# autonomousvision/sdfstudio

Hardware: NVIDIA H100
Metric: rays/sec at 4096 rays x 128 samples (higher is better)
Workload: dtype bf16x3 (fp32 accumulate)

## Files before the change

sdfstudio_b200/csrc/field_tc.h:

```cpp
#pragma once
#include "field_plan.h"

namespace sdfb200 {


constexpr int kEpiWarps = 8;
constexpr int kEpiThreads = kEpiWarps * 32;
constexpr int kTcThreads = kEpiThreads + 128;
constexpr int kEncThreads = 96;
constexpr int kEncItems0 = 288, kEncItems1 = 256, kEncItems2 = 224;
static_assert(kEncItems0 + kEncItems1 + kEncItems2 == 768, "the encoder warps' items cover the tile");
static_assert(kEncItems0 % 32 == 0 && kEncItems1 % 32 == 0, "a warp stages whole 32-row batches (colour_static_tile shuffles across them)");
__host__ __device__ constexpr int enc_item_begin(int w) { return w == 0 ? 0 : w == 1 ? kEncItems0 : w == 2 ? kEncItems0 + kEncItems1 : 768; }
constexpr int kConsumerRegs = 216;
constexpr int kProducerRegs = 72;
static_assert(2 * (kConsumerRegs - 168) <= 168 - kProducerRegs, "setmaxnreg.inc would wait for registers nobody frees");
constexpr int kStages = 5;
constexpr int kKB = 16;
constexpr int kMaxGridDim = 32;
constexpr int kMaxPe = 60;
constexpr int kPeRows = 64;
constexpr int kInK = 96;
constexpr float kHalfPiF = 1.5707963267948966f;
constexpr uint32_t kAPlane = 32 * 2048;
constexpr uint32_t kImgPlane = (kInK / 8) * 128 * 16;
__host__ __device__ constexpr uint32_t tc_stage_bytes(int planes) { return (uint32_t)planes * 256 * kKB * 2; }

enum { PRM_B_G0 = 0, PRM_B_G1, PRM_W_G2 , PRM_B_C0, PRM_B_C1, PRM_W_C2 , kPrmRows = PRM_W_C2 + 3 };
enum { HS_SDF = 0, HS_GRAD , HS_RGB = HS_GRAD + 3 , kHsRows = HS_RGB + 3 };

struct TcSmem { size_t a, ring, prm, hs, coldesc, hx, bytes; };
__host__ __device__ constexpr TcSmem tc_smem(int planes) {
  TcSmem s{};
  s.ring = s.a + (size_t)planes * kAPlane;
  s.prm = s.ring + (size_t)kStages * tc_stage_bytes(planes);
  s.hs = s.prm + kPrmRows * 256 * 4;
  s.coldesc = s.hs + 2 * kHsRows * 128 * 4;
  s.hx = s.coldesc + 96 * 16;
  s.bytes = s.hx + 128 * 8;
  return s;
}
constexpr size_t kSmemPerBlock = 232448;
constexpr size_t kStaticSmem = 1024;
static_assert(tc_smem(2).bytes + kStaticSmem <= kSmemPerBlock, "shared memory of k_field_tc at two planes");

constexpr size_t kFragWords = 64 * 256;
struct TcScratch { size_t sig, h2, slots, slot_bytes, geo, cs, jpe, jg, bytes; };
__host__ __device__ constexpr TcScratch tc_scratch(int planes) {
  TcScratch s{};
  s.h2 = s.sig + kFragWords * 4;
  s.slots = s.h2 + (size_t)planes * kAPlane;
  s.cs = s.geo + (size_t)planes * kImgPlane;
  s.jpe = s.cs + (size_t)planes * kImgPlane;
  s.jg = s.jpe + (size_t)kPeRows * 128 * 4;
  s.slot_bytes = s.jg + (size_t)kMaxGridDim * 3 * 128 * 4;
  s.bytes = s.slots + 2 * s.slot_bytes;
  return s;
}
__host__ __device__ constexpr size_t kScratchPerCta(int planes) { return tc_scratch(planes).bytes; }

__host__ __device__ constexpr int tc_layer_np(int L) { return L == L_B0 ? 128 : 256; }
__host__ __device__ constexpr int tc_layer_k(int L) { return L == L_G0 || L == L_C0MISC ? kInK : 256; }
__host__ __device__ constexpr int tc_layer_kblk(int L) { return kKB * 256 / tc_layer_np(L); }
__host__ __device__ constexpr int tc_layer_nkb(int L) { return tc_layer_k(L) / tc_layer_kblk(L); }
constexpr bool tc_blocks_fill_stages() {
  for (int L = 0; L < L_COUNT; ++L)
    if (tc_layer_np(L) * tc_layer_kblk(L) != 256 * kKB || tc_layer_kblk(L) % 16 != 0 || tc_layer_k(L) % tc_layer_kblk(L) != 0) return false;
  return true;
}
static_assert(tc_blocks_fill_stages(), "every streamed weight block must be one full ring stage of whole K steps");

struct TcLayer {
  unsigned long long w_off;
};

struct TcArgs {
  sdfb200_grid_t grid;
  TcLayer layer[L_COUNT];
// ... 22 lines not shown
```

sdfstudio_b200/csrc/field_tc_kernel.cuh:

```cuda
#pragma once
#include "field_tc.h"
#include "grid.cuh"
#include "tc_common.cuh"

namespace sdfb200 {
using namespace tc;

__device__ __forceinline__ void named_sync(int id, int n) { asm volatile("bar.sync %0, %1;" ::"r"(id), "r"(n) : "memory"); }
constexpr int kEncBar = 3;

struct PointGeom { float px, py, pz, dx, dy, dz, delta, t0, t1; long long ray; };
__device__ __forceinline__ PointGeom point_geom(const TcArgs& a, long long p) {
  PointGeom g;
  g.dx = g.dy = g.dz = 0.f; g.delta = 0.f; g.t0 = g.t1 = 0.f;
  g.ray = a.has_bins ? p / a.n_samples : p;
  if (a.has_bins) {
    const int smp = (int)(p - g.ray * a.n_samples);
    const float t0 = __ldg(a.bins + g.ray * (a.n_samples + 1) + smp);
    g.t0 = t0;
    g.t1 = __ldg(a.bins + g.ray * (a.n_samples + 1) + smp + 1);
    g.delta = __fsub_rn(g.t1, t0);
    g.dx = __ldg(a.directions + g.ray * 3); g.dy = __ldg(a.directions + g.ray * 3 + 1); g.dz = __ldg(a.directions + g.ray * 3 + 2);
    g.px = __fadd_rn(__ldg(a.origins + g.ray * 3 + 0), __fmul_rn(g.dx, t0));
    g.py = __fadd_rn(__ldg(a.origins + g.ray * 3 + 1), __fmul_rn(g.dy, t0));
    g.pz = __fadd_rn(__ldg(a.origins + g.ray * 3 + 2), __fmul_rn(g.dz, t0));
  } else {
    g.px = __ldg(a.origins + p * 3); g.py = __ldg(a.origins + p * 3 + 1); g.pz = __ldg(a.origins + p * 3 + 2);
    if (a.directions) { g.dx = __ldg(a.directions + p * 3); g.dy = __ldg(a.directions + p * 3 + 1); g.dz = __ldg(a.directions + p * 3 + 2); }
  }
  if (a.contraction != SDFB200_CONTRACT_NONE) {
    const float mag = a.contraction == SDFB200_CONTRACT_LINF
                          ? fmaxf(fabsf(g.px), fmaxf(fabsf(g.py), fabsf(g.pz)))
                          : sqrtf(__fadd_rn(__fadd_rn(__fmul_rn(g.px, g.px), __fmul_rn(g.py, g.py)), __fmul_rn(g.pz, g.pz)));
    if (mag >= 1.f) {
      const float k = __fsub_rn(2.f, __fdiv_rn(1.f, mag));
      g.px = __fmul_rn(k, __fdiv_rn(g.px, mag)); g.py = __fmul_rn(k, __fdiv_rn(g.py, mag)); g.pz = __fmul_rn(k, __fdiv_rn(g.pz, mag));
    }
  }
  return g;
}

static __device__ __forceinline__ void sincos_call(float x, float* s, float* c) { sincosf(x, s, c); }
static __device__ __forceinline__ float sin_call(float x) { return sinf(x); }

template <int P, int LAYOUT>
__device__ __forceinline__ void encode_tile_grid(const TcArgs& a, int tile, int row, int grp, uint8_t* img, uint32_t plane, float* Jg,
                                                 uint64_t pol_table) {
  const long long p_raw = (long long)tile * 128 + row;
  const long long p = p_raw < a.n_points ? p_raw : a.n_points - 1;
  const PointGeom g = point_geom(a, p);
  const float x01 = (g.px + 2.0f) * 0.25f, y01 = (g.py + 2.0f) * 0.25f, z01 = (g.pz + 2.0f) * 0.25f;
  const int l_end = min(4 * grp + 4, min(a.grid.n_levels, a.grid.active_levels));
  if (a.use_grid && a.mode != 0) {
#pragma unroll 1
    for (int l = 4 * grp; l < l_end; ++l) {
      LevelCtx c;
      level_prepare<LAYOUT>(a.grid, l, x01, y01, z01, c);
      if (a.grid.table_dtype == SDFB200_DT_F16) level_prefetch_l2<__half, 2>(a.table, c);
      else level_prefetch_l2<float, 2>(a.table, c);
    }
  }
#pragma unroll 1
  for (int l = 4 * grp; l < 4 * grp + 4; ++l) {
    float o[2] = {0.f, 0.f};
    float dj[2][3] = {{0.f, 0.f, 0.f}, {0.f, 0.f, 0.f}};
    if (a.use_grid && l < l_end) {
      LevelCtx c;
      float tv[8][2];
      level_prepare<LAYOUT>(a.grid, l, x01, y01, z01, c);
      if (a.grid.table_dtype == SDFB200_DT_F16) level_fetch<__half, 2, true>(a.table, c, tv, pol_table);
      else level_fetch<float, 2, true>(a.table, c, tv, pol_table);
      level_finish<2, LAYOUT>(a.grid, c, tv, o, dj);
    }
    store_a<P>(img, plane, row, 2 * l, o[0]);
    store_a<P>(img, plane, row, 2 * l + 1, o[1]);
    if (a.mode != 0 && l < a.grid.n_levels) {
#pragma unroll
      for (int f = 0; f < 2; ++f) {
        const int cg = l * 2 + f;
        Jg[(cg * 3 + 0) * 128 + row] = 0.25f * dj[f][0];
        Jg[(cg * 3 + 1) * 128 + row] = 0.25f * dj[f][1];
        Jg[(cg * 3 + 2) * 128 + row] = 0.25f * dj[f][2];
      }
    }
  }
}

template <int P>
__device__ __forceinline__ void encode_tile_pe(const TcArgs& a, int tile, int row, uint8_t* img, uint32_t plane, float* Jpe) {
  const long long p_raw = (long long)tile * 128 + row;
  const long long p = p_raw < a.n_points ? p_raw : a.n_points - 1;
  const PointGeom g = point_geom(a, p);
  if (p_raw < a.n_points) {
    if (a.out.points_norm) a.out.points_norm[p] = sqrtf(__fadd_rn(__fadd_rn(__fmul_rn(g.px, g.px), __fmul_rn(g.py, g.py)), __fmul_rn(g.pz, g.pz)));
    if (a.out.points) { a.out.points[p * 3] = g.px; a.out.points[p * 3 + 1] = g.py; a.out.points[p * 3 + 2] = g.pz; }
  }
  const int deg = a.pe_degree, half = 3 * deg;
  const float pc[3] = {g.px, g.py, g.pz};
  const uint4 z4 = make_uint4(0u, 0u, 0u, 0u);
#pragma unroll 1
  for (int ch = 4; ch < kInK / 8; ++ch) store_a_chunk<P>(img, plane, row, ch, z4, z4);
#pragma unroll 1
  for (int i = 0; i < a.pe_dim; ++i) {
    const int ia = i >= half ? i - half : i;
    const int b = ia / deg, k = ia - b * deg;
    const float fr = (float)(1 << k);
    const float xb = b == 0 ? pc[0] : (b == 1 ? pc[1] : pc[2]);
    const float arg = i >= half ? xb * fr + kHalfPiF : xb * fr;
    float sv, cv;
    sincos_call(arg, &sv, &cv);
    store_a<P>(img, plane, row, 32 + i, a.use_pe ? sv : 0.f);
    if (a.mode != 0) Jpe[i * 128 + row] = a.use_pe ? fr * cv : 0.f;
  }
  store_a<P>(img, plane, row, 32 + a.pe_dim + 0, pc[0]);
  store_a<P>(img, plane, row, 32 + a.pe_dim + 1, pc[1]);
  store_a<P>(img, plane, row, 32 + a.pe_dim + 2, pc[2]);
}

__device__ __forceinline__ float dir_enc(const PointGeom& g, int k) {
  const int i = k < 12 ? k : k - 12, b = i >> 2;
  const float db = b == 0 ? g.dx : (b == 1 ? g.dy : g.dz);
  const float arg = db * (float)(1 << (i & 3));
  return sin_call(k < 12 ? arg : arg + kHalfPiF);
}

template <int P>
__device__ __forceinline__ void colour_static_tile(const TcArgs& a, int tile, int row, uint8_t* img, uint32_t plane) {
  const long long p_raw = (long long)tile * 128 + row;
  const long long p = p_raw < a.n_points ? p_raw : a.n_points - 1;
  const PointGeom g = point_geom(a, p);
  const bool one_ray = __match_any_sync(0xffffffffu, g.ray) == 0xffffffffu;
  const int lane = row & 31;
  const float own = one_ray && lane < 24 ? dir_enc(g, lane) : 0.f;
  const uint4 z4 = make_uint4(0u, 0u, 0u, 0u);
#pragma unroll 1
  for (int ch = 1; ch < kInK / 8; ++ch) store_a_chunk<P>(img, plane, row, ch, z4, z4);
  store_a<P>(img, plane, row, 8 + 0, g.px); store_a<P>(img, plane, row, 8 + 1, g.py); store_a<P>(img, plane, row, 8 + 2, g.pz);
#pragma unroll 1
  for (int k = 0; k < 24; ++k) store_a<P>(img, plane, row, 8 + 3 + k, one_ray ? __shfl_sync(0xffffffffu, own, k) : dir_enc(g, k));
  store_a<P>(img, plane, row, 8 + 27, g.dx); store_a<P>(img, plane, row, 8 + 28, g.dy); store_a<P>(img, plane, row, 8 + 29, g.dz);
  if (a.appearance != nullptr) {
#pragma unroll 1
    for (int j = 0; j < a.app_dim; ++j) store_a<P>(img, plane, row, 8 + 30 + j, __ldg(a.appearance + g.ray * a.app_dim + j));
  }
}

template <int P>
struct Slot {
  uint8_t* base;
  __device__ __forceinline__ Slot(char* slots, uint32_t s) : base(reinterpret_cast<uint8_t*>(slots) + s * tc_scratch(P).slot_bytes) {}
  __device__ __forceinline__ uint8_t* geo() const { return base + tc_scratch(P).geo; }
  __device__ __forceinline__ uint8_t* cs() const { return base + tc_scratch(P).cs; }
  __device__ __forceinline__ float* jpe() const { return reinterpret_cast<float*>(base + tc_scratch(P).jpe); }
  __device__ __forceinline__ float* jg() const { return reinterpret_cast<float*>(base + tc_scratch(P).jg); }
};

#ifdef SDFB200_TC_TIMING
__device__ long long g_tc_timing[16 * 48];
#define TC_PUT(tno, k, v)                                                                                            \
  do {                                                                                                               \
    if (blockIdx.x == 0 && (tno) >= 0 && (tno) < 16) g_tc_timing[(tno) * 48 + (k)] = (v);                            \
  } while (0)
#else
#define TC_PUT(tno, k, v) do { (void)(v); } while (0)
#endif
#define TC_STAMP(k) do { if (tid == 0) TC_PUT(tile_no, k, TC_CLOCK()); } while (0)

struct TcBars {
  Handoff<kStages> ring;
  Handoff<2> enc;
  Handoff<1> a;
  Handoff<2> hs;
  uint64_t cop[2][2];
};

template <int P>
__device__ __forceinline__ void produce_all(const TcArgs& a, int nlayers, uint8_t* abuf, uint8_t* ring, char* slots, TcBars& b) {
  uint32_t j = 0;
// ... 162 lines not shown
    if (c < 3) {
#pragma unroll
      for (int k = 0; k < 16; ++k) sw[k] = sw_next[k];
    }
  }
}

__device__ __forceinline__ float4 col_desc(const TcArgs& a, int ip) {
  const int deg = a.pe_degree, half = 3 * deg;
  int jrow = -1, ax = -1;
  if (ip < a.pe_dim) {
    const int ia = ip >= half ? ip - half : ip;
    ax = ia < deg ? 0 : (ia < 2 * deg ? 1 : 2);
    jrow = ip * 128;
  } else if (ip - a.pe_dim < 3) {
    ax = ip - a.pe_dim;
  }
  return make_float4(__int_as_float(jrow), ax == 0 ? 1.f : 0.f, ax == 1 ? 1.f : 0.f, ax == 2 ? 1.f : 0.f);
}

template <int P>
__device__ __forceinline__ void copy_chunks(uint8_t* abuf, int a_chunk, const uint8_t* src, uint32_t src_plane, int src_chunk, int n, int wrow0,
                                            uint64_t* bar, int lane) {
  for (int k = lane; k < P * n; k += 32) {
    const int pl = k / n, c = k - pl * n;
    bulk_g2s(abuf + pl * kAPlane + (a_chunk + c) * kAChunk + wrow0 * 16, src + pl * src_plane + (src_chunk + c) * kAChunk + wrow0 * 16, 64 * 16, bar);
  }
}
template <int P>
__device__ __forceinline__ void colour_copy(const TileCtx& x, bool early, const uint8_t* cs, uint64_t* bar) {
  constexpr int kMisc = kInK / 8;
  const int lane = x.t & 31;
  if (lane == 0) mbar_arrive_expect_tx(bar, (uint32_t)P * (early ? (kMisc - 1) + kH2Early : 32 - kH2Early) * 64 * 16);
  __syncwarp();
  if (early) {
    copy_chunks<P>(x.abuf, 1, cs, kImgPlane, 1, kMisc - 1, x.wrow0, bar, lane);
    copy_chunks<P>(x.abuf, kMisc, x.h2img, kAPlane, 0, kH2Early, x.wrow0, bar, lane);
  } else {
    copy_chunks<P>(x.abuf, 0, x.h2img, kAPlane, kH2Early, 32 - kH2Early, x.wrow0, bar, lane);
  }
}

template <int P>
__device__ __forceinline__ void epi_eb0(const TileCtx& x, int tile, const Slot<P>& s, const float (&acc)[4][32]) {
  const TcArgs& a = x.a;
  const float* Jpe = s.jpe();
  const float* Jg = s.jg();
  float g0x = 0.f, g0y = 0.f, g0z = 0.f, g1x = 0.f, g1y = 0.f, g1z = 0.f;
#pragma unroll
  for (int c = 0; c < 2; ++c) {
#pragma unroll
    for (int i = 0; i < 32; ++i) {
      const int col = frag_col(x.cq, c, i), row = frag_row(x.r0, i);
      const bool h = frag_half(i);
      float& gx = h ? g1x : g0x;
      float& gy = h ? g1y : g0y;
      float& gz = h ? g1z : g0z;
      const float g = acc[c][i];
      if (c == 0 && i < 16) {
        const bool live = col < a.grid_dim;
        const float* j = Jg + col * 3 * 128 + row;
        const float jx = live ? j[0] : 0.f, jy = live ? j[128] : 0.f, jz = live ? j[256] : 0.f;
        gx = fmaf(g, jx, gx); gy = fmaf(g, jy, gy); gz = fmaf(g, jz, gz);
      } else {
        const float4 d = x.coldesc[col - 32];
        const int jrow = __float_as_int(d.x);
        const float tv = __fmul_rn(g, jrow >= 0 ? Jpe[jrow + row] : 1.f);
        gx = fmaf(tv, d.y, gx); gy = fmaf(tv, d.z, gy); gz = fmaf(tv, d.w, gz);
      }
    }
  }
  g0x = quad_sum(g0x); g0y = quad_sum(g0y); g0z = quad_sum(g0z);
  g1x = quad_sum(g1x); g1y = quad_sum(g1y); g1z = quad_sum(g1z);
  if ((x.t & 3) < 2) {
    const int h = x.t & 1, row = x.r0 + 8 * h;
    const long long p_raw = (long long)tile * 128 + row;
    const PointGeom pg = point_geom(a, p_raw < a.n_points ? p_raw : a.n_points - 1);
    const float grx = h ? g1x : g0x, gry = h ? g1y : g0y, grz = h ? g1z : g0z;
    const float3 n = normalize_eps(grx, gry, grz);
    const float c0v[8] = {grx, gry, grz, a.use_n_dot_v ? n.x * pg.dx + n.y * pg.dy + n.z * pg.dz : 0.f, 0.f, 0.f, 0.f, 0.f};
    store_a_chunk<P>(x.abuf, kAPlane, row, 0, c0v);
    x.hs[HS_GRAD][row] = grx; x.hs[HS_GRAD + 1][row] = gry; x.hs[HS_GRAD + 2][row] = grz;
  }
}

template <int P>
__device__ __forceinline__ void epi_ec0(const TileCtx& x, float (&acc)[4][32]) {
  const float* p_bc0 = x.prm[PRM_B_C0];
#pragma unroll 1
  for (int c = 0; c < 4; ++c, acc_shift(acc)) {
    float2 bias[8];
    load_prm_block(p_bc0, x.cq, c, 0, bias);
#pragma unroll
    for (int i = 0; i < 32; i += 2) {
      const int col = frag_col(x.cq, c, i), row = frag_row(x.r0, i);
      const float2 b2 = bias[i >> 2];
      store_a_pair<P>(x.abuf, kAPlane, row, col, fmaxf(acc[0][i] + b2.x, 0.f), fmaxf(acc[0][i + 1] + b2.y, 0.f));
    }
  }
}

__device__ __forceinline__ void epi_ec1(const TileCtx& x, float (&acc)[4][32]) {
  const float* p_bc1 = x.prm[PRM_B_C1];
// ... 8 lines not shown
      float& rr = h ? r1r : r0r;
      float& rg = h ? r1g : r0g;
      float& rb = h ? r1b : r0b;
      const float v = fmaxf(acc[0][i] + p_bc1[col], 0.f);
      rr = fmaf(p_wc2[0][col], v, rr);
      rg = fmaf(p_wc2[1][col], v, rg);
      rb = fmaf(p_wc2[2][col], v, rb);
    }
  }
  r0r = quad_sum(r0r); r0g = quad_sum(r0g); r0b = quad_sum(r0b);
  r1r = quad_sum(r1r); r1g = quad_sum(r1g); r1b = quad_sum(r1b);
  if ((x.t & 3) < 2) {
    const int h = x.t & 1, row = x.r0 + 8 * h;
    x.hs[HS_RGB][row] = h ? r1r : r0r; x.hs[HS_RGB + 1][row] = h ? r1g : r0g; x.hs[HS_RGB + 2][row] = h ? r1b : r0b;
  }
}

struct HeadsXfer { double wtot[2][4]; float csum[2][4][8]; };
static_assert(sizeof(TcBars) + sizeof(HeadsXfer) <= kStaticSmem, "static shared memory of k_field_tc (kStaticSmem)");
enum { HR_ALPHA = HS_SDF , HR_NORMAL = HS_GRAD , HR_RGB = HS_RGB  };
struct RayEnd { int q; double tot; float last[3]; };
struct HeadsClock { long long rows, scan, sums; };

__device__ __forceinline__ float sample_mid(const TcArgs& a, long long p) {
  if (!a.has_bins) return 0.f;
  const long long ray = p / a.n_samples;
  const float* b = a.bins + ray * (a.n_samples + 1) + (p - ray * a.n_samples);
  return __fdiv_rn(__fadd_rn(__ldg(b), __ldg(b + 1)), 2.0f);
}

__device__ __forceinline__ void heads_rows(const TcArgs& a, float (*hs)[128], double* hx, double* wtot, int tile, int q, int lane,
                                           float& dmin, float& dmax, HeadsClock& clk) {
  long long tc0 = TC_CLOCK();
  const float* b_c2 = reinterpret_cast<const float*>(a.blob + a.b_c2);
  const int row = q * 32 + lane;
  const long long p_raw = (long long)tile * 128 + row;
  const bool valid = p_raw < a.n_points;
  const long long p = valid ? p_raw : a.n_points - 1;
  const PointGeom pg = point_geom(a, p);
  const float dirx = pg.dx, diry = pg.dy, dirz = pg.dz, delta = pg.delta;
  const float sdf = hs[HS_SDF][row], grx = hs[HS_GRAD][row], gry = hs[HS_GRAD + 1][row], grz = hs[HS_GRAD + 2][row];
  const float3 nv = normalize_eps(grx, gry, grz);
  const float nx = nv.x, ny = nv.y, nz = nv.z;
  float rgbv[3];
#pragma unroll
  for (int c = 0; c < 3; ++c) rgbv[c] = padded_rgb(sigmoidf_(hs[HS_RGB + c][row] + __ldg(b_c2 + c)), a.rgb_padding);
  float density = 0.f, alpha = 0.f;
  if (a.out.density || (a.render && a.rnd.from_density)) density = sdf_density(sdf, __ldg(a.beta), __ldg(a.beta_min));
  if (a.out.alpha || (a.render && !a.rnd.from_density))
    alpha = neus_alpha(sdf, dirx * grx + diry * gry + dirz * grz, delta, __ldg(a.variance), a.cos_anneal);
  if (valid) {
    if (a.out.rgb) { a.out.rgb[p * 3] = rgbv[0]; a.out.rgb[p * 3 + 1] = rgbv[1]; a.out.rgb[p * 3 + 2] = rgbv[2]; }
    if (a.out.gradients) { a.out.gradients[p * 3] = grx; a.out.gradients[p * 3 + 1] = gry; a.out.gradients[p * 3 + 2] = grz; }
    if (a.out.normals) { a.out.normals[p * 3] = nx; a.out.normals[p * 3 + 1] = ny; a.out.normals[p * 3 + 2] = nz; }
    if (a.out.density) a.out.density[p] = density;
    if (a.out.occupancy) a.out.occupancy[p] = occupancy(sdf);
    if (a.out.alpha) a.out.alpha[p] = alpha;
  }
  { const long long c = TC_CLOCK(); clk.rows += c - tc0; tc0 = c; }
  if (!a.render) return;
  const int S = a.n_samples;
  const int s_idx = row % S;
// ... 42 lines not shown
    if (a.rnd.bg_transmittance) a.rnd.bg_transmittance[ray] = dens ? expf(-(float)tot) : (float)tot;
  }
  clk.sums += TC_CLOCK() - tc0;
}

__device__ __forceinline__ void composite_chunk(const TcArgs& a, const float (*hs)[128], const double* hx, const double* wtot, float (*csum)[8],
                                                int tile, int q, int lane, RayEnd& end, HeadsClock& clk) {
  long long tc0 = TC_CLOCK();
  const int row = q * 32 + lane;
  const long long p_raw = (long long)tile * 128 + row;
  const bool valid = p_raw < a.n_points;
  const long long p = valid ? p_raw : a.n_points - 1;
  const int S = a.n_samples;
  const bool dens = a.rnd.from_density != 0;
  const int first = (q * 32 / S) * (S / 32);
  double excl = hx[row];
  for (int w2 = first; w2 < q; ++w2) excl = dens ? excl + wtot[w2] : excl * wtot[w2];
  const float T = dens ? expf(-(float)excl) : (float)excl;
  const float w = valid ? __fmul_rn(hs[HR_ALPHA][row], T) : 0.f;
  if (valid && a.rnd.weights) a.rnd.weights[p] = w;
  { const long long c = TC_CLOCK(); clk.scan += c - tc0; tc0 = c; }
  const float rgbv[3] = {hs[HR_RGB][row], hs[HR_RGB + 1][row], hs[HR_RGB + 2][row]};
  float vs[8] = {w, w * rgbv[0], w * rgbv[1], w * rgbv[2], w * hs[HR_NORMAL][row], w * hs[HR_NORMAL + 1][row], w * hs[HR_NORMAL + 2][row],
                 w * sample_mid(a, p)};
#pragma unroll
  for (int d = 1; d < 32; d <<= 1) {
#pragma unroll
    for (int k = 0; k < 8; ++k) vs[k] += __shfl_down_sync(0xffffffffu, vs[k], d);
  }
  if (lane == 0) {
#pragma unroll
    for (int k = 0; k < 8; ++k) csum[q][k] = vs[k];
  }
  if (q == first + S / 32 - 1) {
    end.q = q;
    if (dens) {
      end.tot = __shfl_sync(0xffffffffu, excl, 31);
    } else {
      end.tot = 1.0;
      for (int w2 = first; w2 <= q; ++w2) end.tot *= wtot[w2];
    }
#pragma unroll
    for (int c = 0; c < 3; ++c) end.last[c] = __shfl_sync(0xffffffffu, rgbv[c], 31);
  }
  clk.sums += TC_CLOCK() - tc0;
}

__device__ __forceinline__ void finish_rays(const TcArgs& a, const float (*csum)[8], int tile, int lane, const RayEnd& end, HeadsClock& clk) {
  const long long tc0 = TC_CLOCK();
  const int S = a.n_samples;
  const long long ray = (long long)tile * (128 / S) + end.q * 32 / S;
  if (end.q >= 0 && lane == 0 && ray * S < a.n_points) {
    float s[8] = {0.f, 0.f, 0.f, 0.f, 0.f, 0.f, 0.f, 0.f};
    for (int w2 = end.q + 1 - S / 32; w2 <= end.q; ++w2) {
#pragma unroll
      for (int k = 0; k < 8; ++k) s[k] += csum[w2][k];
    }
    finish_ray(ray, s[0], {s[1], s[2], s[3]}, {s[4], s[5], s[6]}, s[7], a.rnd.bg_mode, a.rnd.bg, end.last, a.rnd.clamp01, a.rnd.out.rgb,
               a.rnd.out.accumulation, a.rnd.out.normal, a.rnd.out.depth);
    const bool dens = a.rnd.from_density != 0;
    if (a.rnd.bg_transmittance) a.rnd.bg_transmittance[ray] = dens ? expf(-(float)end.tot) : (float)end.tot;
  }
  clk.sums += TC_CLOCK() - tc0;
}

__device__ __forceinline__ void heads_of(const TcArgs& a, int tile, int tile_no, int et, TcBars& b, float (*hs)[128], double* hx, HeadsXfer& xf,
                                         float& dmin, float& dmax) {
  const int ew = et >> 5, lane = et & 31;
  long long waited = 0, bar_waited = 0;
  b.hs.wait_full(tile_no, &waited);
  const long long t0 = TC_CLOCK();
  float (*h)[128] = hs + b.hs.slot(tile_no) * kHsRows;
  double* wtot = xf.wtot[tile_no & 1];
  float (*csum)[8] = xf.csum[tile_no & 1];
  HeadsClock clk{0, 0, 0};
#pragma unroll 1
  for (int q = ew; q < 4; q += kEncThreads / 32) heads_rows(a, h, hx, wtot, tile, q, lane, dmin, dmax, clk);
  if (a.render && a.n_samples > 32) {
    long long c = TC_CLOCK();
    named_sync(kEncBar, kEncThreads);
    bar_waited += TC_CLOCK() - c;
    RayEnd end{-1, 0.0, {0.f, 0.f, 0.f}};
#pragma unroll 1
    for (int q = ew; q < 4; q += kEncThreads / 32) composite_chunk(a, h, hx, wtot, csum, tile, q, lane, end, clk);
    c = TC_CLOCK();
    named_sync(kEncBar, kEncThreads);
    bar_waited += TC_CLOCK() - c;
    finish_rays(a, csum, tile, lane, end, clk);
  }
  b.hs.arrive_empty(tile_no);
  if (lane == 0) TC_PUT(tile_no, ew == 0 ? 14 : 25 + ew, TC_CLOCK() - t0);
  if (et == 0) { TC_PUT(tile_no, 17, waited); TC_PUT(tile_no, 28, clk.rows); TC_PUT(tile_no, 29, clk.scan); TC_PUT(tile_no, 30, clk.sums); TC_PUT(tile_no, 31, bar_waited); }
}

template <int P, int LAYOUT>
__device__ __forceinline__ void encode_all(const TcArgs& a, int et, char* slots, TcBars& b, uint64_t pol_table, float (*hs)[128], double* hx,
                                           HeadsXfer& xf) {
  const bool heads = a.mode != 0;
  const int ew = et >> 5, lane = et & 31;
  const int i_begin = heads ? enc_item_begin(ew) + lane : et, i_end = heads ? enc_item_begin(ew + 1) : 640, i_step = heads ? 32 : kEncThreads;
  float dmin = INFINITY, dmax = -INFINITY;
  int tile_no = 0;
  for (int tile = blockIdx.x; tile < a.n_tiles; tile += gridDim.x, ++tile_no) {
    long long waited = 0;
    b.enc.wait_empty(tile_no, &waited);
    const long long t0 = TC_CLOCK();
    const Slot<P> s(slots, b.enc.slot(tile_no));
    long long kind_grid = 0, kind_pe = 0, kind_cs = 0;
#pragma unroll 1
    for (int i = i_begin; i < i_end; i += i_step) {
      const int row = i & 127;
      const long long c0 = TC_CLOCK();
      if (i < 512) { encode_tile_grid<P, LAYOUT>(a, tile, row, i >> 7, s.geo(), kImgPlane, s.jg(), pol_table); kind_grid += TC_CLOCK() - c0; }
      else if (i < 640) { encode_tile_pe<P>(a, tile, row, s.geo(), kImgPlane, s.jpe()); kind_pe += TC_CLOCK() - c0; }
      else { colour_static_tile<P>(a, tile, row, s.cs(), kImgPlane); kind_cs += TC_CLOCK() - c0; }
    }
    fence_async_global();
    b.enc.arrive_full(tile_no);
    if (et == 0) { TC_PUT(tile_no, 12, TC_CLOCK() - t0); TC_PUT(tile_no, 13, waited); }
    else if (lane == 0) TC_PUT(tile_no, 23 + ew, TC_CLOCK() - t0);
    if (lane == 0) { TC_PUT(tile_no, 32 + 3 * ew, kind_grid); TC_PUT(tile_no, 33 + 3 * ew, kind_pe); TC_PUT(tile_no, 34 + 3 * ew, kind_cs); }
    if (heads && tile_no > 0) heads_of(a, tile - (int)gridDim.x, tile_no - 1, et, b, hs, hx, xf, dmin, dmax);
  }
  if (heads && tile_no > 0) heads_of(a, blockIdx.x + (tile_no - 1) * (int)gridDim.x, tile_no - 1, et, b, hs, hx, xf, dmin, dmax);
  if (heads && a.render && a.rnd.out.steps_minmax) {
#pragma unroll
    for (int d = 1; d < 32; d <<= 1) {
      dmin = fminf(dmin, __shfl_xor_sync(0xffffffffu, dmin, d));
      dmax = fmaxf(dmax, __shfl_xor_sync(0xffffffffu, dmax, d));
    }
    if (lane == 0 && dmin <= dmax) { atomic_min_float(a.rnd.out.steps_minmax, dmin); atomic_max_float(a.rnd.out.steps_minmax + 1, dmax); }
  }
}

template <int P, int LAYOUT>
__global__ void __launch_bounds__(kTcThreads, 1) k_field_tc(const __grid_constant__ TcArgs a) {
  extern __shared__ __align__(1024) uint8_t smem[];
  constexpr TcSmem sm = tc_smem(P);
  constexpr TcScratch scr = tc_scratch(P);
  uint8_t* abuf = smem + sm.a;
  uint8_t* ring = smem + sm.ring;
  float (*prm)[256] = reinterpret_cast<float (*)[256]>(smem + sm.prm);
  float (*hs)[128] = reinterpret_cast<float (*)[128]>(smem + sm.hs);
  float4* coldesc = reinterpret_cast<float4*>(smem + sm.coldesc);
  double* hx = reinterpret_cast<double*>(smem + sm.hx);
  __shared__ TcBars bars;
  __shared__ HeadsXfer hxf;

  const int tid = threadIdx.x, warp = tid >> 5, lane = tid & 31;
  const int nlayers = a.mode == 0 ? 2 : L_COUNT;
  char* cta_scr = a.scratch + (size_t)blockIdx.x * scr.bytes;
  char* slots = cta_scr + scr.slots;
  if (tid == 0) {
    bars.ring.init(1, kEpiWarps);
    bars.enc.init(kEncThreads, kEpiThreads);
    bars.hs.init(kEpiThreads, kEncThreads);
    bars.a.init(1, 2);
    for (int w = 0; w < 2; ++w) { mbar_init(&bars.cop[w][0], 1); mbar_init(&bars.cop[w][1], 1); }
    fence_barrier_init();
  }
  {
    const char* blob = a.blob;
    const float* src[kPrmRows] = {reinterpret_cast<const float*>(blob + a.b_g0), reinterpret_cast<const float*>(blob + a.b_g1),
                                  reinterpret_cast<const float*>(blob + a.w_g2), reinterpret_cast<const float*>(blob + a.b_c0),
                                  reinterpret_cast<const float*>(blob + a.b_c1), reinterpret_cast<const float*>(blob + a.w_c2),
                                  reinterpret_cast<const float*>(blob + a.w_c2) + 256, reinterpret_cast<const float*>(blob + a.w_c2) + 512};
    for (int i = tid; i < kPrmRows * 256; i += kTcThreads) prm[i >> 8][i & 255] = src[i >> 8][i & 255];
    if (tid < 96) coldesc[tid] = col_desc(a, tid);
  }
  __syncthreads();

  if (tid >= kEpiThreads) {
    setmaxnreg_dec<kProducerRegs>();
    if (tid == kEpiThreads) produce_all<P>(a, nlayers, abuf, ring, slots, bars);
    else if (tid >= kTcThreads - kEncThreads) encode_all<P, LAYOUT>(a, tid - (kTcThreads - kEncThreads), slots, bars, l2_policy_evict_last(), hs, hx, hxf);
    return;
  }
  setmaxnreg_inc<kConsumerRegs>();

  const int wg = warp >> 2, t = tid & 127;
  const int wrow0 = wg * 64;
  const int wg_bar = 1 + wg;
  const uint32_t a_base = smem_u32(abuf) + wrow0 * 16;
  const float sdf_bias = __ldg(reinterpret_cast<const float*>(a.blob + a.b_g2));
  TileCtx x{a, tid, t, wg, wrow0, frag_row0(wrow0, t), frag_cq(t), abuf, prm, hs, coldesc, sdf_bias,
            reinterpret_cast<uint32_t*>(cta_scr + scr.sig), reinterpret_cast<uint8_t*>(cta_scr + scr.h2), slots};
  uint32_t it = 0;
  long long waited = 0;
  float acc[4][32];
#define SYNC_A()                \
  do {                          \
    fence_async_smem();         \
    named_sync(wg_bar, 128);    \
  } while (0)
#define LAYER(L, zero)                                                                                 \
  do {                                                                                                 \
    layer_mma<P, L>(acc, zero, a_base, ring, bars.ring, it, lane, waited, &bars.cop[wg][1], tile_no & 1); \
    named_sync(wg_bar, 128);   \
// ... 14 lines not shown
    epi_e0<P>(x, acc);
    TC_STAMP(18);
    SYNC_A();
    LAYER(L_G1, true);
    if (a.mode == 0) {
      if (t == 0) bars.a.arrive_empty(tile_no);
      epi_e1<P>(x, tile, acc);
      continue;
    }
    {
      long long hs_waited = 0;
      bars.hs.wait_empty(tile_no, &hs_waited);
      if (tid == 0) TC_PUT(tile_no, 16, hs_waited);
    }
    epi_e1<P>(x, tile, acc);
    TC_STAMP(19);
    SYNC_A();
    LAYER(L_B1, true);
    epi_eb1<P>(x, acc);
    TC_STAMP(20);
    SYNC_A();
    LAYER(L_B0, true);
    bars.enc.wait_full(tile_no);
    if (t < 32) colour_copy<P>(x, true, s.cs(), &bars.cop[wg][0]);
    epi_eb0<P>(x, tile, s, acc);
    mbar_wait(&bars.cop[wg][0], tile_no & 1);
    bars.enc.arrive_empty(tile_no);
    TC_STAMP(21);
    SYNC_A();
    LAYER(L_C0MISC, true);
    if (t < 32) colour_copy<P>(x, false, nullptr, &bars.cop[wg][1]);
    TC_STAMP(22);
    LAYER(L_C0H, false);
    epi_ec0<P>(x, acc);
    TC_STAMP(23);
    SYNC_A();
    LAYER(L_C1, true);
    if (t == 0) bars.a.arrive_empty(tile_no);
    epi_ec1(x, acc);
    bars.hs.arrive_full(tile_no);
    TC_STAMP(15);
    if (tid == 0) TC_PUT(tile_no, 9, waited);
  }
#undef SYNC_A
#undef LAYER
}

template <int P, int LAYOUT>
static int launch_field_tc(const TcArgs& a, int grid, size_t smem, cudaStream_t st) {
  SDFB_CUDA(cudaFuncSetAttribute(k_field_tc<P, LAYOUT>, cudaFuncAttributeMaxDynamicSharedMemorySize, (int)smem));
  k_field_tc<P, LAYOUT><<<grid, kTcThreads, smem, st>>>(a);
  SDFB_LAUNCHED("k_field_tc");
  return 0;
}
// ... 3 lines not shown
```

Measured before the change: 1.459 million.

## Stage per-tile point geometry once in scratch and batch grid feature stores

The encoder warps now compute each point's position, direction and ray index once per tile into a per-slot scratch area. After a named barrier, the grid, PE, colour-static and epilogue paths read these staged values instead of recomputing point_geom with its bin, origin and direction loads and divides. Grid level outputs are packed into a single 16-byte chunk store per group instead of per-element stores. Warp-uniform role dispatch and bounded bulk-copy loops are also added. The cost is extra scratch memory, an additional encoder barrier per tile, and a new bin indexing path that must match the previous per-point division.

```diff
diff --git a/sdfstudio_b200/csrc/field_tc.h b/sdfstudio_b200/csrc/field_tc.h
--- a/sdfstudio_b200/csrc/field_tc.h
+++ b/sdfstudio_b200/csrc/field_tc.h
@@ -28,6 +28,7 @@
 
 enum { PRM_B_G0 = 0, PRM_B_G1, PRM_W_G2 , PRM_B_C0, PRM_B_C1, PRM_W_C2 , kPrmRows = PRM_W_C2 + 3 };
 enum { HS_SDF = 0, HS_GRAD , HS_RGB = HS_GRAD + 3 , kHsRows = HS_RGB + 3 };
+enum { GEOM_PX = 0, GEOM_PY, GEOM_PZ, GEOM_DX, GEOM_DY, GEOM_DZ, kGeomRows };
 
 struct TcSmem { size_t a, ring, prm, hs, coldesc, hx, bytes; };
 __host__ __device__ constexpr TcSmem tc_smem(int planes) {
@@ -45,7 +46,7 @@
 static_assert(tc_smem(2).bytes + kStaticSmem <= kSmemPerBlock, "shared memory of k_field_tc at two planes");
 
 constexpr size_t kFragWords = 64 * 256;
-struct TcScratch { size_t sig, h2, slots, slot_bytes, geo, cs, jpe, jg, bytes; };
+struct TcScratch { size_t sig, h2, slots, slot_bytes, geo, cs, jpe, jg, geom, ray, bytes; };
 __host__ __device__ constexpr TcScratch tc_scratch(int planes) {
   TcScratch s{};
   s.h2 = s.sig + kFragWords * 4;
@@ -53,7 +54,9 @@
   s.cs = s.geo + (size_t)planes * kImgPlane;
   s.jpe = s.cs + (size_t)planes * kImgPlane;
   s.jg = s.jpe + (size_t)kPeRows * 128 * 4;
-  s.slot_bytes = s.jg + (size_t)kMaxGridDim * 3 * 128 * 4;
+  s.geom = s.jg + (size_t)kMaxGridDim * 3 * 128 * 4;
+  s.ray = s.geom + (size_t)kGeomRows * 128 * 4;
+  s.slot_bytes = s.ray + 128 * 8;
   s.bytes = s.slots + 2 * s.slot_bytes;
   return s;
 }
diff --git a/sdfstudio_b200/csrc/field_tc_kernel.cuh b/sdfstudio_b200/csrc/field_tc_kernel.cuh
--- a/sdfstudio_b200/csrc/field_tc_kernel.cuh
+++ b/sdfstudio_b200/csrc/field_tc_kernel.cuh
@@ -9,16 +9,25 @@
 __device__ __forceinline__ void named_sync(int id, int n) { asm volatile("bar.sync %0, %1;" ::"r"(id), "r"(n) : "memory"); }
 constexpr int kEncBar = 3;
 
+__device__ __forceinline__ const float* point_bin(const TcArgs& a, int tile, int row, long long& ray) {
+  const long long p0 = (long long)tile * 128;
+  const long long ray0 = p0 / a.n_samples;
+  const int s = (int)(p0 - ray0 * a.n_samples) + (int)(min(p0 + row, a.n_points - 1) - p0);
+  ray = ray0 + s / a.n_samples;
+  return a.bins + ray * (a.n_samples + 1) + s % a.n_samples;
+}
+
 struct PointGeom { float px, py, pz, dx, dy, dz, delta, t0, t1; long long ray; };
-__device__ __forceinline__ PointGeom point_geom(const TcArgs& a, long long p) {
+__device__ __forceinline__ PointGeom point_geom(const TcArgs& a, int tile, int row) {
+  const long long p = min((long long)tile * 128 + row, a.n_points - 1);
   PointGeom g;
   g.dx = g.dy = g.dz = 0.f; g.delta = 0.f; g.t0 = g.t1 = 0.f;
-  g.ray = a.has_bins ? p / a.n_samples : p;
+  g.ray = p;
   if (a.has_bins) {
-    const int smp = (int)(p - g.ray * a.n_samples);
-    const float t0 = __ldg(a.bins + g.ray * (a.n_samples + 1) + smp);
+    const float* bin = point_bin(a, tile, row, g.ray);
+    const float t0 = __ldg(bin);
     g.t0 = t0;
-    g.t1 = __ldg(a.bins + g.ray * (a.n_samples + 1) + smp + 1);
+    g.t1 = __ldg(bin + 1);
     g.delta = __fsub_rn(g.t1, t0);
     g.dx = __ldg(a.directions + g.ray * 3); g.dy = __ldg(a.directions + g.ray * 3 + 1); g.dz = __ldg(a.directions + g.ray * 3 + 2);
     g.px = __fadd_rn(__ldg(a.origins + g.ray * 3 + 0), __fmul_rn(g.dx, t0));
@@ -43,13 +52,35 @@
 static __device__ __forceinline__ void sincos_call(float x, float* s, float* c) { sincosf(x, s, c); }
 static __device__ __forceinline__ float sin_call(float x) { return sinf(x); }
 
+template <int P>
+struct Slot {
+  uint8_t* base;
+  __device__ __forceinline__ Slot(char* slots, uint32_t s) : base(reinterpret_cast<uint8_t*>(slots) + s * tc_scratch(P).slot_bytes) {}
+  __device__ __forceinline__ uint8_t* geo() const { return base + tc_scratch(P).geo; }
+  __device__ __forceinline__ uint8_t* cs() const { return base + tc_scratch(P).cs; }
+  __device__ __forceinline__ float* jpe() const { return reinterpret_cast<float*>(base + tc_scratch(P).jpe); }
+  __device__ __forceinline__ float* jg() const { return reinterpret_cast<float*>(base + tc_scratch(P).jg); }
+  __device__ __forceinline__ float (*geom() const)[128] { return reinterpret_cast<float (*)[128]>(base + tc_scratch(P).geom); }
+  __device__ __forceinline__ long long* ray() const { return reinterpret_cast<long long*>(base + tc_scratch(P).ray); }
+};
+
+template <int P>
+__device__ __forceinline__ void stage_geom(const TcArgs& a, int tile, int et, const Slot<P>& s) {
+  float (*gm)[128] = s.geom();
+#pragma unroll 1
+  for (int row = et; row < 128; row += kEncThreads) {
+    const PointGeom g = point_geom(a, tile, row);
+    gm[GEOM_PX][row] = g.px; gm[GEOM_PY][row] = g.py; gm[GEOM_PZ][row] = g.pz;
+    gm[GEOM_DX][row] = g.dx; gm[GEOM_DY][row] = g.dy; gm[GEOM_DZ][row] = g.dz;
+    s.ray()[row] = g.ray;
+  }
+}
+
 template <int P, int LAYOUT>
-__device__ __forceinline__ void encode_tile_grid(const TcArgs& a, int tile, int row, int grp, uint8_t* img, uint32_t plane, float* Jg,
-                                                 uint64_t pol_table) {
-  const long long p_raw = (long long)tile * 128 + row;
-  const long long p = p_raw < a.n_points ? p_raw : a.n_points - 1;
-  const PointGeom g = point_geom(a, p);
-  const float x01 = (g.px + 2.0f) * 0.25f, y01 = (g.py + 2.0f) * 0.25f, z01 = (g.pz + 2.0f) * 0.25f;
+__device__ __forceinline__ void encode_tile_grid(const TcArgs& a, int row, int grp, const Slot<P>& s, uint64_t pol_table) {
+  const float (*gm)[128] = s.geom();
+  float* Jg = s.jg();
+  const float x01 = (gm[GEOM_PX][row] + 2.0f) * 0.25f, y01 = (gm[GEOM_PY][row] + 2.0f) * 0.25f, z01 = (gm[GEOM_PZ][row] + 2.0f) * 0.25f;
   const int l_end = min(4 * grp + 4, min(a.grid.n_levels, a.grid.active_levels));
   if (a.use_grid && a.mode != 0) {
 #pragma unroll 1
@@ -60,6 +91,7 @@
       else level_prefetch_l2<float, 2>(a.table, c);
     }
   }
+  uint32_t h0 = 0u, h1 = 0u, h2 = 0u, h3 = 0u, l0 = 0u, l1 = 0u, l2 = 0u, l3 = 0u;
 #pragma unroll 1
   for (int l = 4 * grp; l < 4 * grp + 4; ++l) {
     float o[2] = {0.f, 0.f};
@@ -72,8 +104,10 @@
       else level_fetch<float, 2, true>(a.table, c, tv, pol_table);
       level_finish<2, LAYOUT>(a.grid, c, tv, o, dj);
     }
-    store_a<P>(img, plane, row, 2 * l, o[0]);
-    store_a<P>(img, plane, row, 2 * l + 1, o[1]);
+    uint32_t hi, lo;
+    split2(o[0], o[1], hi, lo);
+    h0 = h1; h1 = h2; h2 = h3; h3 = hi;
+    l0 = l1; l1 = l2; l2 = l3; l3 = lo;
     if (a.mode != 0 && l < a.grid.n_levels) {
 #pragma unroll
       for (int f = 0; f < 2; ++f) {
@@ -84,76 +118,73 @@
       }
     }
   }
-}
-
-template <int P>
-__device__ __forceinline__ void encode_tile_pe(const TcArgs& a, int tile, int row, uint8_t* img, uint32_t plane, float* Jpe) {
-  const long long p_raw = (long long)tile * 128 + row;
-  const long long p = p_raw < a.n_points ? p_raw : a.n_points - 1;
-  const PointGeom g = point_geom(a, p);
-  if (p_raw < a.n_points) {
-    if (a.out.points_norm) a.out.points_norm[p] = sqrtf(__fadd_rn(__fadd_rn(__fmul_rn(g.px, g.px), __fmul_rn(g.py, g.py)), __fmul_rn(g.pz, g.pz)));
-    if (a.out.points) { a.out.points[p * 3] = g.px; a.out.points[p * 3 + 1] = g.py; a.out.points[p * 3 + 2] = g.pz; }
+  store_a_chunk<P>(s.geo(), kImgPlane, row, grp, make_uint4(h0, h1, h2, h3), make_uint4(l0, l1, l2, l3));
+}
+
+template <int P>
+__device__ __forceinline__ void encode_tile_pe(const TcArgs& a, int tile, int row, const Slot<P>& s) {
+  const long long p = (long long)tile * 128 + row;
+  const float (*gm)[128] = s.geom();
+  const float px = gm[GEOM_PX][row], py = gm[GEOM_PY][row], pz = gm[GEOM_PZ][row];
+  if (p < a.n_points) {
+    if (a.out.points_norm) a.out.points_norm[p] = sqrtf(__fadd_rn(__fadd_rn(__fmul_rn(px, px), __fmul_rn(py, py)), __fmul_rn(pz, pz)));
+    if (a.out.points) { a.out.points[p * 3] = px; a.out.points[p * 3 + 1] = py; a.out.points[p * 3 + 2] = pz; }
   }
   const int deg = a.pe_degree, half = 3 * deg;
-  const float pc[3] = {g.px, g.py, g.pz};
+  uint8_t* img = s.geo();
+  float* Jpe = s.jpe();
   const uint4 z4 = make_uint4(0u, 0u, 0u, 0u);
 #pragma unroll 1
-  for (int ch = 4; ch < kInK / 8; ++ch) store_a_chunk<P>(img, plane, row, ch, z4, z4);
+  for (int ch = 4; ch < kInK / 8; ++ch) store_a_chunk<P>(img, kImgPlane, row, ch, z4, z4);
 #pragma unroll 1
   for (int i = 0; i < a.pe_dim; ++i) {
     const int ia = i >= half ? i - half : i;
     const int b = ia / deg, k = ia - b * deg;
     const float fr = (float)(1 << k);
-    const float xb = b == 0 ? pc[0] : (b == 1 ? pc[1] : pc[2]);
+    const float xb = b == 0 ? px : (b == 1 ? py : pz);
     const float arg = i >= half ? xb * fr + kHalfPiF : xb * fr;
     float sv, cv;
     sincos_call(arg, &sv, &cv);
-    store_a<P>(img, plane, row, 32 + i, a.use_pe ? sv : 0.f);
+    store_a<P>(img, kImgPlane, row, 32 + i, a.use_pe ? sv : 0.f);
     if (a.mode != 0) Jpe[i * 128 + row] = a.use_pe ? fr * cv : 0.f;
   }
-  store_a<P>(img, plane, row, 32 + a.pe_dim + 0, pc[0]);
-  store_a<P>(img, plane, row, 32 + a.pe_dim + 1, pc[1]);
-  store_a<P>(img, plane, row, 32 + a.pe_dim + 2, pc[2]);
-}
-
-__device__ __forceinline__ float dir_enc(const PointGeom& g, int k) {
+  store_a<P>(img, kImgPlane, row, 32 + a.pe_dim + 0, px);
+  store_a<P>(img, kImgPlane, row, 32 + a.pe_dim + 1, py);
+  store_a<P>(img, kImgPlane, row, 32 + a.pe_dim + 2, pz);
+}
+
+__device__ __forceinline__ float dir_enc(float dx, float dy, float dz, int k) {
   const int i = k < 12 ? k : k - 12, b = i >> 2;
-  const float db = b == 0 ? g.dx : (b == 1 ? g.dy : g.dz);
+  const float db = b == 0 ? dx : (b == 1 ? dy : dz);
   const float arg = db * (float)(1 << (i & 3));
   return sin_call(k < 12 ? arg : arg + kHalfPiF);
 }
 
 template <int P>
-__device__ __forceinline__ void colour_static_tile(const TcArgs& a, int tile, int row, uint8_t* img, uint32_t plane) {
-  const long long p_raw = (long long)tile * 128 + row;
-  const long long p = p_raw < a.n_points ? p_raw : a.n_points - 1;
-  const PointGeom g = point_geom(a, p);
-  const bool one_ray = __match_any_sync(0xffffffffu, g.ray) == 0xffffffffu;
+__device__ __forceinline__ void colour_static_tile(const TcArgs& a, int row, const Slot<P>& s) {
+  const float (*gm)[128] = s.geom();
+  const float px = gm[GEOM_PX][row], py = gm[GEOM_PY][row], pz = gm[GEOM_PZ][row];
+  const float dx = gm[GEOM_DX][row], dy = gm[GEOM_DY][row], dz = gm[GEOM_DZ][row];
+  const long long ray = s.ray()[row];
+  const bool one_ray = __match_any_sync(0xffffffffu, ray) == 0xffffffffu;
   const int lane = row & 31;
-  const float own = one_ray && lane < 24 ? dir_enc(g, lane) : 0.f;
+  const float own = one_ray && lane < 24 ? dir_enc(dx, dy, dz, lane) : 0.f;
+  uint8_t* img = s.cs();
   const uint4 z4 = make_uint4(0u, 0u, 0u, 0u);
 #pragma unroll 1
-  for (int ch = 1; ch < kInK / 8; ++ch) store_a_chunk<P>(img, plane, row, ch, z4, z4);
-  store_a<P>(img, plane, row, 8 + 0, g.px); store_a<P>(img, plane, row, 8 + 1, g.py); store_a<P>(img, plane, row, 8 + 2, g.pz);
-#pragma unroll 1
-  for (int k = 0; k < 24; ++k) store_a<P>(img, plane, row, 8 + 3 + k, one_ray ? __shfl_sync(0xffffffffu, own, k) : dir_enc(g, k));
-  store_a<P>(img, plane, row, 8 + 27, g.dx); store_a<P>(img, plane, row, 8 + 28, g.dy); store_a<P>(img, plane, row, 8 + 29, g.dz);
+  for (int ch = 1; ch < kInK / 8; ++ch) store_a_chunk<P>(img, kImgPlane, row, ch, z4, z4);
+  store_a<P>(img, kImgPlane, row, 8 + 0, px); store_a<P>(img, kImgPlane, row, 8 + 1, py); store_a<P>(img, kImgPlane, row, 8 + 2, pz);
+#pragma unroll 1
+  for (int k = 0; k < 24; ++k) {
+    const float shared = __shfl_sync(0xffffffffu, own, k);
+    store_a<P>(img, kImgPlane, row, 8 + 3 + k, one_ray ? shared : dir_enc(dx, dy, dz, k));
+  }
+  store_a<P>(img, kImgPlane, row, 8 + 27, dx); store_a<P>(img, kImgPlane, row, 8 + 28, dy); store_a<P>(img, kImgPlane, row, 8 + 29, dz);
   if (a.appearance != nullptr) {
 #pragma unroll 1
-    for (int j = 0; j < a.app_dim; ++j) store_a<P>(img, plane, row, 8 + 30 + j, __ldg(a.appearance + g.ray * a.app_dim + j));
-  }
-}
-
-template <int P>
-struct Slot {
-  uint8_t* base;
-  __device__ __forceinline__ Slot(char* slots, uint32_t s) : base(reinterpret_cast<uint8_t*>(slots) + s * tc_scratch(P).slot_bytes) {}
-  __device__ __forceinline__ uint8_t* geo() const { return base + tc_scratch(P).geo; }
-  __device__ __forceinline__ uint8_t* cs() const { return base + tc_scratch(P).cs; }
-  __device__ __forceinline__ float* jpe() const { return reinterpret_cast<float*>(base + tc_scratch(P).jpe); }
-  __device__ __forceinline__ float* jg() const { return reinterpret_cast<float*>(base + tc_scratch(P).jg); }
-};
+    for (int j = 0; j < a.app_dim; ++j) store_a<P>(img, kImgPlane, row, 8 + 30 + j, __ldg(a.appearance + ray * a.app_dim + j));
+  }
+}
 
 #ifdef SDFB200_TC_TIMING
 __device__ long long g_tc_timing[16 * 48];
@@ -362,9 +393,12 @@
 template <int P>
 __device__ __forceinline__ void copy_chunks(uint8_t* abuf, int a_chunk, const uint8_t* src, uint32_t src_plane, int src_chunk, int n, int wrow0,
                                             uint64_t* bar, int lane) {
-  for (int k = lane; k < P * n; k += 32) {
-    const int pl = k / n, c = k - pl * n;
-    bulk_g2s(abuf + pl * kAPlane + (a_chunk + c) * kAChunk + wrow0 * 16, src + pl * src_plane + (src_chunk + c) * kAChunk + wrow0 * 16, 64 * 16, bar);
+  for (int k0 = 0; k0 < P * n; k0 += 32) {
+    const int k = k0 + lane;
+    if (k < P * n) {
+      const int pl = k / n, c = k - pl * n;
+      bulk_g2s(abuf + pl * kAPlane + (a_chunk + c) * kAChunk + wrow0 * 16, src + pl * src_plane + (src_chunk + c) * kAChunk + wrow0 * 16, 64 * 16, bar);
+    }
   }
 }
 template <int P>
@@ -382,7 +416,7 @@
 }
 
 template <int P>
-__device__ __forceinline__ void epi_eb0(const TileCtx& x, int tile, const Slot<P>& s, const float (&acc)[4][32]) {
+__device__ __forceinline__ void epi_eb0(const TileCtx& x, const Slot<P>& s, const float (&acc)[4][32]) {
   const TcArgs& a = x.a;
   const float* Jpe = s.jpe();
   const float* Jg = s.jg();
@@ -414,11 +448,11 @@
   g1x = quad_sum(g1x); g1y = quad_sum(g1y); g1z = quad_sum(g1z);
   if ((x.t & 3) < 2) {
     const int h = x.t & 1, row = x.r0 + 8 * h;
-    const long long p_raw = (long long)tile * 128 + row;
-    const PointGeom pg = point_geom(a, p_raw < a.n_points ? p_raw : a.n_points - 1);
+    const float (*gm)[128] = s.geom();
     const float grx = h ? g1x : g0x, gry = h ? g1y : g0y, grz = h ? g1z : g0z;
     const float3 n = normalize_eps(grx, gry, grz);
-    const float c0v[8] = {grx, gry, grz, a.use_n_dot_v ? n.x * pg.dx + n.y * pg.dy + n.z * pg.dz : 0.f, 0.f, 0.f, 0.f, 0.f};
+    const float c0v[8] = {grx, gry, grz, a.use_n_dot_v ? n.x * gm[GEOM_DX][row] + n.y * gm[GEOM_DY][row] + n.z * gm[GEOM_DZ][row] : 0.f,
+                          0.f, 0.f, 0.f, 0.f};
     store_a_chunk<P>(x.abuf, kAPlane, row, 0, c0v);
     x.hs[HS_GRAD][row] = grx; x.hs[HS_GRAD + 1][row] = gry; x.hs[HS_GRAD + 2][row] = grz;
   }
@@ -473,10 +507,10 @@
 struct RayEnd { int q; double tot; float last[3]; };
 struct HeadsClock { long long rows, scan, sums; };
 
-__device__ __forceinline__ float sample_mid(const TcArgs& a, long long p) {
+__device__ __forceinline__ float sample_mid(const TcArgs& a, int tile, int row) {
   if (!a.has_bins) return 0.f;
-  const long long ray = p / a.n_samples;
-  const float* b = a.bins + ray * (a.n_samples + 1) + (p - ray * a.n_samples);
+  long long ray;
+  const float* b = point_bin(a, tile, row, ray);
   return __fdiv_rn(__fadd_rn(__ldg(b), __ldg(b + 1)), 2.0f);
 }
 
@@ -488,7 +522,7 @@
   const long long p_raw = (long long)tile * 128 + row;
   const bool valid = p_raw < a.n_points;
   const long long p = valid ? p_raw : a.n_points - 1;
-  const PointGeom pg = point_geom(a, p);
+  const PointGeom pg = point_geom(a, tile, row);
   const float dirx = pg.dx, diry = pg.dy, dirz = pg.dz, delta = pg.delta;
   const float sdf = hs[HS_SDF][row], grx = hs[HS_GRAD][row], gry = hs[HS_GRAD + 1][row], grz = hs[HS_GRAD + 2][row];
   const float3 nv = normalize_eps(grx, gry, grz);
@@ -577,7 +611,7 @@
   { const long long c = TC_CLOCK(); clk.scan += c - tc0; tc0 = c; }
   const float rgbv[3] = {hs[HR_RGB][row], hs[HR_RGB + 1][row], hs[HR_RGB + 2][row]};
   float vs[8] = {w, w * rgbv[0], w * rgbv[1], w * rgbv[2], w * hs[HR_NORMAL][row], w * hs[HR_NORMAL + 1][row], w * hs[HR_NORMAL + 2][row],
-                 w * sample_mid(a, p)};
+                 w * sample_mid(a, tile, row)};
 #pragma unroll
   for (int d = 1; d < 32; d <<= 1) {
 #pragma unroll
@@ -619,9 +653,8 @@
   clk.sums += TC_CLOCK() - tc0;
 }
 
-__device__ __forceinline__ void heads_of(const TcArgs& a, int tile, int tile_no, int et, TcBars& b, float (*hs)[128], double* hx, HeadsXfer& xf,
-                                         float& dmin, float& dmax) {
-  const int ew = et >> 5, lane = et & 31;
+__device__ __forceinline__ void heads_of(const TcArgs& a, int tile, int tile_no, int ew, int lane, TcBars& b, float (*hs)[128], double* hx,
+                                         HeadsXfer& xf, float& dmin, float& dmax) {
   long long waited = 0, bar_waited = 0;
   b.hs.wait_full(tile_no, &waited);
   const long long t0 = TC_CLOCK();
@@ -645,15 +678,15 @@
   }
   b.hs.arrive_empty(tile_no);
   if (lane == 0) TC_PUT(tile_no, ew == 0 ? 14 : 25 + ew, TC_CLOCK() - t0);
-  if (et == 0) { TC_PUT(tile_no, 17, waited); TC_PUT(tile_no, 28, clk.rows); TC_PUT(tile_no, 29, clk.scan); TC_PUT(tile_no, 30, clk.sums); TC_PUT(tile_no, 31, bar_waited); }
+  if (ew == 0 && lane == 0) { TC_PUT(tile_no, 17, waited); TC_PUT(tile_no, 28, clk.rows); TC_PUT(tile_no, 29, clk.scan); TC_PUT(tile_no, 30, clk.sums); TC_PUT(tile_no, 31, bar_waited); }
 }
 
 template <int P, int LAYOUT>
-__device__ __forceinline__ void encode_all(const TcArgs& a, int et, char* slots, TcBars& b, uint64_t pol_table, float (*hs)[128], double* hx,
-                                           HeadsXfer& xf) {
+__device__ __forceinline__ void encode_all(const TcArgs& a, int ew, int lane, char* slots, TcBars& b, uint64_t pol_table, float (*hs)[128],
+                                           double* hx, HeadsXfer& xf) {
   const bool heads = a.mode != 0;
-  const int ew = et >> 5, lane = et & 31;
-  const int i_begin = heads ? enc_item_begin(ew) + lane : et, i_end = heads ? enc_item_begin(ew + 1) : 640, i_step = heads ? 32 : kEncThreads;
+  const int et = ew * 32 + lane;
+  const int i_begin = heads ? enc_item_begin(ew) : ew * 32, i_end = heads ? enc_item_begin(ew + 1) : 640, i_step = heads ? 32 : kEncThreads;
   float dmin = INFINITY, dmax = -INFINITY;
   int tile_no = 0;
   for (int tile = blockIdx.x; tile < a.n_tiles; tile += gridDim.x, ++tile_no) {
@@ -661,23 +694,29 @@
     b.enc.wait_empty(tile_no, &waited);
     const long long t0 = TC_CLOCK();
     const Slot<P> s(slots, b.enc.slot(tile_no));
-    long long kind_grid = 0, kind_pe = 0, kind_cs = 0;
-#pragma unroll 1
-    for (int i = i_begin; i < i_end; i += i_step) {
-      const int row = i & 127;
+    long long kind_grid = 0, kind_pe = 0, kind_cs = 0, geom = 0;
+    stage_geom<P>(a, tile, et, s);
+    named_sync(kEncBar, kEncThreads);
+    geom = TC_CLOCK() - t0;
+#pragma unroll 1
+    for (int ib = i_begin; ib < i_end; ib += i_step) {
+      const int row = (ib & 127) + lane;
       const long long c0 = TC_CLOCK();
-      if (i < 512) { encode_tile_grid<P, LAYOUT>(a, tile, row, i >> 7, s.geo(), kImgPlane, s.jg(), pol_table); kind_grid += TC_CLOCK() - c0; }
-      else if (i < 640) { encode_tile_pe<P>(a, tile, row, s.geo(), kImgPlane, s.jpe()); kind_pe += TC_CLOCK() - c0; }
-      else { colour_static_tile<P>(a, tile, row, s.cs(), kImgPlane); kind_cs += TC_CLOCK() - c0; }
+      if (ib < 512) { encode_tile_grid<P, LAYOUT>(a, row, ib >> 7, s, pol_table); kind_grid += TC_CLOCK() - c0; }
+      else if (ib < 640) { encode_tile_pe<P>(a, tile, row, s); kind_pe += TC_CLOCK() - c0; }
+      else { colour_static_tile<P>(a, row, s); kind_cs += TC_CLOCK() - c0; }
     }
     fence_async_global();
     b.enc.arrive_full(tile_no);
     if (et == 0) { TC_PUT(tile_no, 12, TC_CLOCK() - t0); TC_PUT(tile_no, 13, waited); }
     else if (lane == 0) TC_PUT(tile_no, 23 + ew, TC_CLOCK() - t0);
-    if (lane == 0) { TC_PUT(tile_no, 32 + 3 * ew, kind_grid); TC_PUT(tile_no, 33 + 3 * ew, kind_pe); TC_PUT(tile_no, 34 + 3 * ew, kind_cs); }
-    if (heads && tile_no > 0) heads_of(a, tile - (int)gridDim.x, tile_no - 1, et, b, hs, hx, xf, dmin, dmax);
-  }
-  if (heads && tile_no > 0) heads_of(a, blockIdx.x + (tile_no - 1) * (int)gridDim.x, tile_no - 1, et, b, hs, hx, xf, dmin, dmax);
+    if (lane == 0) {
+      TC_PUT(tile_no, 32 + 3 * ew, kind_grid); TC_PUT(tile_no, 33 + 3 * ew, kind_pe); TC_PUT(tile_no, 34 + 3 * ew, kind_cs);
+      TC_PUT(tile_no, 41 + ew, geom);
+    }
+    if (heads && tile_no > 0) heads_of(a, tile - (int)gridDim.x, tile_no - 1, ew, lane, b, hs, hx, xf, dmin, dmax);
+  }
+  if (heads && tile_no > 0) heads_of(a, blockIdx.x + (tile_no - 1) * (int)gridDim.x, tile_no - 1, ew, lane, b, hs, hx, xf, dmin, dmax);
   if (heads && a.render && a.rnd.out.steps_minmax) {
 #pragma unroll
     for (int d = 1; d < 32; d <<= 1) {
@@ -702,7 +741,7 @@
   __shared__ TcBars bars;
   __shared__ HeadsXfer hxf;
 
-  const int tid = threadIdx.x, warp = tid >> 5, lane = tid & 31;
+  const int tid = threadIdx.x, warp = __shfl_sync(0xffffffffu, tid >> 5, 0), lane = tid & 31;
   const int nlayers = a.mode == 0 ? 2 : L_COUNT;
   char* cta_scr = a.scratch + (size_t)blockIdx.x * scr.bytes;
   char* slots = cta_scr + scr.slots;
@@ -725,10 +764,14 @@
   }
   __syncthreads();
 
-  if (tid >= kEpiThreads) {
+  constexpr int kEncWarp0 = (kTcThreads - kEncThreads) / 32;
+  if (warp >= kEpiWarps) {
     setmaxnreg_dec<kProducerRegs>();
-    if (tid == kEpiThreads) produce_all<P>(a, nlayers, abuf, ring, slots, bars);
-    else if (tid >= kTcThreads - kEncThreads) encode_all<P, LAYOUT>(a, tid - (kTcThreads - kEncThreads), slots, bars, l2_policy_evict_last(), hs, hx, hxf);
+    if (warp == kEpiWarps) {
+      if (lane == 0) produce_all<P>(a, nlayers, abuf, ring, slots, bars);
+    } else if (warp >= kEncWarp0) {
+      encode_all<P, LAYOUT>(a, warp - kEncWarp0, lane, slots, bars, l2_policy_evict_last(), hs, hx, hxf);
+    }
     return;
   }
   setmaxnreg_inc<kConsumerRegs>();
@@ -789,14 +832,14 @@
     SYNC_A();
     LAYER(L_B0, true);
     bars.enc.wait_full(tile_no);
-    if (t < 32) colour_copy<P>(x, true, s.cs(), &bars.cop[wg][0]);
-    epi_eb0<P>(x, tile, s, acc);
+    if ((warp & 3) == 0) colour_copy<P>(x, true, s.cs(), &bars.cop[wg][0]);
+    epi_eb0<P>(x, s, acc);
     mbar_wait(&bars.cop[wg][0], tile_no & 1);
     bars.enc.arrive_empty(tile_no);
     TC_STAMP(21);
     SYNC_A();
     LAYER(L_C0MISC, true);
-    if (t < 32) colour_copy<P>(x, false, nullptr, &bars.cop[wg][1]);
+    if ((warp & 3) == 0) colour_copy<P>(x, false, nullptr, &bars.cop[wg][1]);
     TC_STAMP(22);
     LAYER(L_C0H, false);
     epi_ec0<P>(x, acc);
```

Result: faster. 1.542 million, median of 6 (+5.7%).
